# fgiral000/gencast-flax-nnx

Hardware: AMD Instinct MI355X
Metric: denoiser-calls/sec (higher is better)
Workload: dtype f16x3 (every product = 3 fp16 MFMAs on hi/lo-split f32 operands: 22-bit products, f32 accumulate; f32 storage); 1 GPU; nano-GenCast DPM-Solver++2S 20-step sample, 2.5deg grid (73x144), 1 ensemble member per GPU, batch 1; dead_call_skipped=True, grid_nodes=10512, mesh_nodes=2562, latent=256, layers=16, heads=4, ffw_hidden=2048, c_in=262, c_out=82, k_hop=8, parallelism=ensemble-dp1, broadcast=none, rccl_ranks=0, precision=f16x3, library_built_from_this_tree=True, launcher=single

## Files before the change

### gencast-flax-nnx_amd/csrc/gc_api.hip

```cpp
#include <hip/hip_runtime.h>

#include <array>
#include <cmath>
#include <cstdio>
#include <cstdlib>
#include <cstring>
#include <map>
#include <memory>
#include <mutex>
#include <string>
#include <vector>

#include <dlfcn.h>
#include <rccl/rccl.h>

#include "../../include/gencast_hip.h"
#include "../../include/gencast_hip_debug.h"
#include "gc_graph.h"
#include "gc_kernels.h"

template <class To, class From>
static const To& a16_view(const From& v) {
  static_assert(sizeof(To) == sizeof(From), "argument struct mismatch between the two kernel builds");
  return reinterpret_cast<const To&>(v);
// ... 75 lines not shown
  DevMlp m2g_embed_edge, m2g_edge, m2g_grid, m2g_dec;
  std::vector<DevLayer> layers;
  int cond_final = -1;
  int cond_total = 0;
  std::map<std::string, std::pair<int, int>> cond_sites;
  float *d_nw0t = nullptr, *d_nb0 = nullptr, *d_nw1t = nullptr, *d_nb1 = nullptr;
  float *d_wc_all = nullptr, *d_bc_all = nullptr;

  float *d_m0_hat = nullptr, *d_e0_hat = nullptr, *d_f0_hat = nullptr;

  int kp = 0;
  float *d_sigma = nullptr, *d_condvec = nullptr, *d_cond = nullptr;
  float* d_cond_all = nullptr;
  size_t cond_all_cap = 0;
  const float* cond_cur = nullptr;
  float *d_feats = nullptr, *d_xp = nullptr, *d_g0 = nullptr, *d_g1 = nullptr, *d_m0 = nullptr,
        *d_x = nullptr, *d_e1 = nullptr, *d_agg1 = nullptr, *d_qkv = nullptr, *d_att = nullptr,
        *d_u = nullptr, *d_m2 = nullptr, *d_f1 = nullptr, *d_agg2 = nullptr, *d_g2 = nullptr,
        *d_y = nullptr, *d_h = nullptr, *d_part = nullptr, *d_apart_o = nullptr, *d_apart_ml = nullptr,
        *d_pg = nullptr, *d_pm = nullptr;
  bool mlp_ws = true;
  bool mlp_pair = true;
  bool embed_cache = true;
  bool embed_cache_ready = false;
  bool embed_cache_live = false;
  int nwp = 0;
  float *d_xn = nullptr, *d_pstat = nullptr;
  float *w1st_t = nullptr, *w1st_s = nullptr;
  DevMlp g2m_embed_grid_n;
  std::vector<int> h_slots;
  int64_t embed_cache_samples = 0;
  bool mlp_ws512 = true;
  bool m2g_fuse_sum = true;
  bool last_m2g_fused = false;
  float *d_ones = nullptr, *d_zeros = nullptr;
  int hidden_layers = 1;
  float* d_mlp_tmp[2] = {nullptr, nullptr};
  float *d_feats2 = nullptr, *d_ro_a = nullptr, *d_ro_b = nullptr, *d_ro_forc = nullptr;
  int *d_ro_kind = nullptr, *d_ro_src = nullptr, *d_ro_sidx = nullptr;
  int ro_nforc = -1, ro_forc_cap = 0;
  bool has_sample = false;
  int max_tile_chunks = 0;
  int ffw_fused_slabs = 0;
  int ws_mt = 0;
  bool attn_f16 = true;
  bool attn_v2 = true;
  void* d_kv16 = nullptr;
  bool attn_v2_force = false;
  bool kv16_live = false;
  bool fuse_outrow = true;
  bool gemm_ws = true;
  bool f32_ws = true;
  int ffw_xcd = 0;
  bool fuse_combine = true;
  bool split_edge = false;
  int attn_splits = 1, out_splits = 1, ffw2_splits = 1;
  bool a16 = true;
  bool st16 = false;
  bool last_st16 = false;
  int wt_stores = 0;
  int mt_qkv = 1, mt_out = 1, mt_ffw1 = 1, mt_ffw2 = 1;
  int* d_slots = nullptr;
  float *d_sx = nullptr, *d_sden = nullptr, *d_smid = nullptr, *d_noise = nullptr;
  float *d_noise_alt = nullptr, *last_noise = nullptr;
  float* d_stash = nullptr;
  hipEvent_t ev_stash = nullptr;
  bool has_stash = false;

  int nz_L = 0, nz_lat = 0, nz_lon = 0;
  float *d_nz_leg = nullptr, *d_nz_cos = nullptr, *d_nz_sin = nullptr, *d_nz_coef = nullptr, *d_nz_f = nullptr;
  unsigned long long nz_key = 0, nz_stream = 0;
  std::vector<float> churn_rates;
  float churn_inflation = 1.0f;

  struct SampleGraph {
    std::vector<float> sigmas;
    int skip_dead = 1;
    const float* noise = nullptr;
    bool f16 = false, feat16 = false, st16 = false;
    hipGraph_t graph = nullptr;
    hipGraphExec_t exec = nullptr, exec2 = nullptr;
    hipEvent_t done[2] = {nullptr, nullptr};
    int next = 0;
    int calls = 0;
    int64_t launches_per_call = 0, launches = 0;
    uint64_t last_use = 0;
  };
  bool use_graphs = true;
  std::vector<SampleGraph> sample_graphs;
  uint64_t graph_clock = 0;
  int64_t graph_replays = 0, graph_captures = 0;
  int debug_layer_limit = -1;
  int debug_stop_layer = -1, debug_stop_phase = -1;
  bool f16x3 = true;
  float g2m_agg_norm = 0.f;
  bool feat16 = false;
  bool weights_f16_unsafe = false;
  bool in_fallback = false;
  unsigned* d_nonfinite = nullptr;
  unsigned* h_nonfinite = nullptr;
  unsigned nonfinite_seen = 0;
  int64_t range_fallbacks = 0;
  bool guard_pending = false;
  std::vector<float> last_sigmas;
  int last_skip_dead = 1;
  unsigned long long last_stream0 = 0;
// ... 721 lines not shown
      return rc;
    }
    const bool fuse_combine = h->attn_splits > 1 && h->attn_splits <= 8 && h->mt_out == 1 && h->fuse_combine;
    if (h->attn_splits > 1 && !fuse_combine && (rc = launch(h, gc::KC_ATTN_COMBINE, [&] {
          return gc::launch_attn_combine(s, h->d_apart_o, h->d_apart_ml, g.M, B, D, c.num_heads,
                                         h->attn_splits, h->d_att, false, h->feat16);
        })))
      return rc;
    const bool fuse_row = (f16 || x32) && h->gemm_ws && h->fuse_outrow && D % 128 == 0 && D <= 512 &&
                          (h->attn_splits == 1 || fuse_combine);
    if (fuse_row) {
      gc::GemmArgs ga{};
      ga.a = h->d_att; ga.lda = D; ga.a_f32 = 1; ga.wt = x32 ? ly.wo_x : ly.wo_f; ga.ldw = D; ga.rows = MB; ga.n = D; ga.k_slice = D;
      ga.f32w = x32 ? 1 : 0;
      if (h->attn_splits > 1) {
        ga.att_po = h->d_apart_o; ga.att_pml = h->d_apart_ml; ga.att_S = h->attn_splits; ga.att_B = B;
        ga.att_H = c.num_heads; ga.att_DH = D / c.num_heads;
      } else if (use_items) {
        ga.att_po = h->d_apart_o; ga.att_pml = h->d_apart_ml; ga.att_S = 0; ga.att_B = B;
        ga.att_H = c.num_heads; ga.att_DH = D / c.num_heads; ga.att_tiles = h->d_att_tiles;
      }
      ga.round16 = h->feat16 ? 1 : 0; ga.a16 = st16 ? 1 : 0;
      gc::RowFuse rf{h->d_x, ly.bo, cond + ly.cond_ffw, cs, B, h->d_h, h->feat16 ? 1 : 0};
      if ((rc = launch(h, gc::KC_GEMM_OUT, [&] {
             return ga.a16 ? gc_a16::launch_gemm_rowop(s, gc::KC_GEMM_OUT, a16_view<gc_a16::GemmArgs>(ga),
                                                       a16_view<gc_a16::RowFuse>(rf))
                           : gc::launch_gemm_rowop(s, gc::KC_GEMM_OUT, ga, rf);
           })))
        return rc;
    } else if (fuse_combine) {
      gc::GemmArgs ga{};
      const bool ws = use_ws(D, D, h->out_splits);
      ga.a = h->d_att; ga.lda = D; ga.a_f32 = 1; ga.wt = ws ? (x32 ? ly.wo_x : ly.wo_f) : (f16 ? ly.wo_s : ly.wo_t); ga.ldw = D; ga.rows = MB;
      ga.f32w = (ws && x32) ? 1 : 0;
      ga.n = D; ga.k_slice = D / h->out_splits; ga.out = h->d_part; ga.ldo = D;
      ga.att_po = h->d_apart_o; ga.att_pml = h->d_apart_ml; ga.att_S = h->attn_splits; ga.att_B = B;
      ga.att_H = c.num_heads; ga.att_DH = D / c.num_heads; ga.round16 = h->feat16 ? 1 : 0; ga.a16 = st16 ? 1 : 0;
      if ((rc = launch(h, gc::KC_GEMM_OUT, [&] {
             return ws ? (ga.a16 ? gc_a16::launch_gemm_ws(s, gc::KC_GEMM_OUT, a16_view<gc_a16::GemmArgs>(ga), 1, h->out_splits, 1)
                                 : gc::launch_gemm_ws(s, gc::KC_GEMM_OUT, ga, 1, h->out_splits, 1))
                       : gc::launch_gemm(s, gc::KC_GEMM_OUT, ga, 1, h->out_splits, 1, f16);
           })))
        return rc;
    } else if ((rc = gemm(gc::KC_GEMM_OUT, h->d_att, D, f16 ? ly.wo_s : ly.wo_t, x32 ? ly.wo_x : ly.wo_f, D, D, D, h->out_splits,
                          nullptr, 0, h->d_part, D, h->mt_out, 1)))
      return rc;
    if (!fuse_row && (rc = rowop(ly.bo, h->out_splits, ly.cond_ffw, h->d_h))) return rc;
    if (stop_here(i, 2)) return GC_OK;
    if (ffw_slabs > 0) {
      gc::FfwArgs fa{h->d_h, MB, (int)D, (int)F, x32 ? ly.w1_x : ly.w1_f, ly.b1, x32 ? ly.w2_x : ly.w2_f, h->d_part,
                     h->feat16 ? 1 : 0, h->wt_stores & 1, st16 ? 1 : 0};
      fa.f32w = x32 ? 1 : 0;
      fa.xcd_tiles = (h->ffw_xcd && D == 256) ? 1 : 0;
      if ((rc = launch(h, gc::KC_GEMM_FFW1, [&] {
             return fa.a16 ? gc_a16::launch_ffw_fused(s, a16_view<gc_a16::FfwArgs>(fa)) : gc::launch_ffw_fused(s, fa);
           })))
        return rc;
    } else {
    if ((rc = gemm(gc::KC_GEMM_FFW1, h->d_h, D, f16 ? ly.w1_s : ly.w1_t, x32 ? ly.w1_x : ly.w1_f, D, F, D, 1, ly.b1, 1, h->d_u, F,
                   h->mt_ffw1, 0)))
      return rc;
    if ((rc = gemm(gc::KC_GEMM_FFW2, h->d_u, F, f16 ? ly.w2_s : ly.w2_t, x32 ? ly.w2_x : ly.w2_f, F, D, F, h->ffw2_splits, nullptr, 0,
                   h->d_part, D, h->mt_ffw2, 1)))
      return rc;
    }
    pend_bias = ly.b2;
    pend_slabs = ffw_slabs > 0 ? ffw_slabs : h->ffw2_splits;
  }
  if ((rc = rowop(pend_bias, pend_slabs, h->cond_final, h->d_m2))) return rc;

  if (side) GC_HIP(h, hipStreamWaitEvent(s, h->ev_join, 0));
  if (h->split_edge) {
    if ((rc = node_gemm(h->d_m2, g.M * B, h->m2g_edge.w1snd_t, h->m2g_edge.w1snd_s, h->m2g_edge.w1snd_f, h->d_pm))) return rc;
    if ((rc = node_gemm(h->d_g1, g.G * B, h->m2g_edge.w1rcv_t, h->m2g_edge.w1rcv_s, h->m2g_edge.w1rcv_f, h->d_pg))) return rc;
  }
  const bool fuse_sum = m2g_sum_fusable(h);
  h->last_m2g_fused = fuse_sum;
  if ((rc = run_m2g_edge(h, cond, fuse_sum))) return rc;
  if (!fuse_sum && (rc = launch(h, gc::KC_SEGSUM, [&] {
         return gc::launch_segsum(s, h->d_f1, h->d_m2g_ptr, h->d_m2g_eid, g.G, g.E2, B, L, h->d_agg2, h->feat16, st16);
       })))
    return rc;
  if ((rc = run_mlp(h, h->m2g_grid,
                    {seg(h->d_g1, nullptr, nullptr, L, L, 0), seg(h->d_agg2, nullptr, nullptr, L, L, 0)},
                    g.G * B, B, true, true, h->d_g1, h->d_g2, L)))
    return rc;
  if ((rc = run_mlp(h, h->m2g_dec, {seg(h->d_g2, nullptr, nullptr, L, L, 0)}, g.G * B, B, false, false,
                    nullptr, h->d_y, c.c_out, nullptr, nullptr, true, nullptr, false, true)))
    return rc;
  h->launches_last_call = h->launch_count - launches0;
  return GC_OK;
}

int guard_enqueue(gc_handle* h, const float* p, size_t n) {
  if (!use_f16(h)) return GC_OK;
  int rc = launch(h, gc::KC_PACK, [&] { return gc::launch_finite_check(h->stream, p, n, h->d_nonfinite); });
  if (rc) return rc;
  GC_HIP(h, hipMemcpyAsync(h->h_nonfinite, h->d_nonfinite, sizeof(unsigned), hipMemcpyDeviceToHost, h->stream));
  return GC_OK;
}
bool guard_tripped(gc_handle* h) {
  if (*h->h_nonfinite == h->nonfinite_seen) return false;
  h->nonfinite_seen = *h->h_nonfinite;
  return true;
}

// ... 631 lines not shown
    for (int k = 0; k < 4; ++k) e1s[(size_t)e * 32 + k] = g2m_edge_struct[(size_t)e * 4 + k];
  for (int e = 0; e < E2; ++e)
    for (int k = 0; k < 4; ++k) e2s[(size_t)e * 32 + k] = m2g_edge_struct[(size_t)g.m2g_order[e] * 4 + k];
  if ((rc = dev_upload(h, &h->d_mesh_struct16, ms16))) return rc;
  if ((rc = dev_upload(h, &h->d_e1_struct16, e1s))) return rc;
  if ((rc = dev_upload(h, &h->d_e2_struct16, e2s))) return rc;

  const gc_config& c = h->cfg;
  const size_t B = c.batch, L = c.latent_size, D = c.d_model, F = c.ffw_hidden;
  const size_t GB = (size_t)G * B, MB = (size_t)M * B;
  if ((rc = dev_alloc(h, &h->d_sigma, B))) return rc;
  if ((rc = dev_alloc(h, &h->d_condvec, B * gc::kCondDim))) return rc;
  if ((rc = dev_alloc(h, &h->d_feats, GB * c.c_in))) return rc;
  if ((rc = dev_alloc(h, &h->d_xp, GB * h->kp))) return rc;
  if ((rc = dev_alloc(h, &h->d_g0, GB * L))) return rc;
  if ((rc = dev_alloc(h, &h->d_g1, GB * L))) return rc;
  if ((rc = dev_alloc(h, &h->d_g2, GB * L))) return rc;
  if ((rc = dev_alloc(h, &h->d_agg2, GB * L))) return rc;
  if ((rc = dev_alloc(h, &h->d_m0, MB * L))) return rc;
  if ((rc = dev_alloc(h, &h->d_x, MB * L))) return rc;
  if ((rc = dev_alloc(h, &h->d_agg1, MB * L))) return rc;
  if ((rc = dev_alloc(h, &h->d_m2, MB * L))) return rc;
  if ((rc = dev_alloc(h, &h->d_qkv, MB * 3 * D))) return rc;
  if ((rc = dev_alloc(h, &h->d_att, MB * D))) return rc;
  {
    uint16_t* kv = nullptr;
    if ((rc = dev_alloc(h, &kv, MB * 4 * D))) return rc;
    h->d_kv16 = kv;
  }
  if ((rc = dev_alloc(h, &h->d_u, MB * F))) return rc;
  {
    auto env_int = [](const char* name, int dflt) {
      const char* v = std::getenv(name);
      return (v && *v) ? std::atoi(v) : dflt;
    };
    auto largest_split = [](int k, int cap) {
      int best = 1;
      for (int sp = 1; sp <= cap; ++sp)
        if (k % (32 * sp) == 0) best = sp;
      return best;
    };
    int as = (int)std::lround(256.0 / std::max(1, h->hg.n_tiles * (int)B));
    h->attn_splits = std::min(8, std::max(1, env_int("GC_TUNE_ATTN_SPLITS", as)));
    const int ffw2_wgs = (int)((MB + 63) / 64) * (int)(D / 128);
    h->ffw2_splits = largest_split((int)F, std::max(1, env_int("GC_TUNE_FFW2_SPLITS", ffw2_wgs >= 512 ? 1 : 4)));
    h->out_splits = largest_split((int)D, std::max(1, env_int("GC_TUNE_OUT_SPLITS", 2)));
    h->mt_qkv = env_int("GC_TUNE_MT_QKV", 1) == 2 ? 2 : 1;
    h->mt_out = env_int("GC_TUNE_MT_OUT", 1) == 2 ? 2 : 1;
    h->mt_ffw1 = env_int("GC_TUNE_MT_FFW1", 1) == 2 ? 2 : 1;
    h->mt_ffw2 = env_int("GC_TUNE_MT_FFW2", 1) == 2 ? 2 : 1;
    h->fuse_combine = env_int("GC_TUNE_FUSE_COMBINE", 1) != 0;
    h->gemm_ws = env_int("GC_TUNE_GEMM_WS", 1) != 0;
    h->ffw_xcd = env_int("GC_TUNE_FFW_XCD", 0);
    h->f32_ws = env_int("GC_TUNE_F32_WS", 1) != 0 && h->gemm_ws && D % 128 == 0 && F % 256 == 0;
    h->fuse_outrow = env_int("GC_TUNE_FUSE_OUTROW", 1) != 0;
    h->attn_f16 = env_int("GC_TUNE_ATTN_F16", 1) != 0;
    h->attn_v2 = env_int("GC_TUNE_ATTN_V2", 1) != 0;
    h->fuse_noisy = env_int("GC_TUNE_FUSE_NOISY", 1) != 0;
    h->side_stream = env_int("GC_TUNE_SIDE_STREAM", 0) != 0;
    h->wt_stores = env_int("GC_TUNE_WT_STORES", 0);
    h->a16 = env_int("GC_TUNE_A16", 1) != 0;
    h->attn_v2_force = env_int("GC_TUNE_ATTN_V2", 1) == 2;
    h->ws_mt = env_int("GC_TUNE_WS_MT", 0);
    h->mlp_ws = env_int("GC_TUNE_MLP_WS", 1) != 0;
    h->mlp_ws512 = env_int("GC_TUNE_MLP_WS512", 2) != 0;
    h->m2g_fuse_sum = env_int("GC_TUNE_M2G_FUSE_SUM", 1) != 0;
    h->embed_cache = env_int("GC_TUNE_EMBED_CACHE", 1) != 0;
    h->mlp_pair = env_int("GC_TUNE_MLP_PAIR", 1) != 0;
    const int want_fused = env_int("GC_TUNE_FFW_FUSED", 1);
    h->ffw_fused_slabs = (h->gemm_ws && want_fused != 0 && D % 128 == 0 && (D <= 256 || (want_fused == 2 && D <= 512)) &&
                          F % 256 == 0 && F / 256 <= 16) ? (int)(F / 256) : 0;
    const size_t slabs = (size_t)std::max(std::max(h->ffw2_splits, h->out_splits), std::max(h->ffw_fused_slabs, 1));
    if ((rc = dev_alloc(h, &h->d_h, MB * D))) return rc;
    if ((rc = dev_alloc(h, &h->d_pg, GB * L))) return rc;
    if ((rc = dev_alloc(h, &h->d_pm, MB * L))) return rc;
    if (!h->d_ones) {
      if ((rc = dev_upload(h, &h->d_ones, std::vector<float>(2048, 1.0f)))) return rc;
      if ((rc = dev_upload(h, &h->d_zeros, std::vector<float>(2048, 0.0f)))) return rc;
    }
    h->split_edge = env_int("GC_TUNE_SPLIT_EDGE", L >= 512 ? 1 : 0) != 0;
    if ((rc = dev_alloc(h, &h->d_part, slabs * MB * D))) return rc;
    const size_t aslots = (size_t)h->hg.n_tiles * h->attn_splits * B * c.num_heads;
    if ((rc = dev_alloc(h, &h->d_apart_o, aslots * 32 * (D / c.num_heads)))) return rc;
    if ((rc = dev_alloc(h, &h->d_apart_ml, aslots * 32 * 2))) return rc;
  }
  if ((rc = dev_alloc(h, &h->d_e1, (size_t)E1 * B * L))) return rc;
  if ((rc = dev_alloc(h, &h->d_f1, (size_t)E2 * B * L))) return rc;
  if ((rc = dev_alloc(h, &h->d_y, GB * c.c_out))) return rc;
  if ((rc = dev_alloc(h, &h->d_sx, GB * c.c_out))) return rc;
  if ((rc = dev_alloc(h, &h->d_sden, GB * c.c_out))) return rc;
  if ((rc = dev_alloc(h, &h->d_smid, GB * c.c_out))) return rc;
  if ((rc = dev_alloc(h, &h->d_noise, GB * c.c_out))) return rc;
  if ((rc = dev_alloc(h, &h->d_noise_alt, GB * c.c_out))) return rc;
  if ((rc = dev_alloc(h, &h->d_slots, (size_t)c.c_out))) return rc;
  if ((rc = dev_alloc(h, &h->d_m0_hat, (size_t)M * L))) return rc;
  if ((rc = dev_alloc(h, &h->d_e0_hat, (size_t)E1 * L))) return rc;
  if ((rc = dev_alloc(h, &h->d_f0_hat, (size_t)E2 * L))) return rc;
  GC_HIP(h, hipMemset(h->d_xp, 0, GB * h->kp * sizeof(float)));
  GC_HIP(h, hipHostMalloc((void**)&h->pin_cond, GB * c.c_in * sizeof(float), hipHostMallocDefault));
  GC_HIP(h, hipHostMalloc((void**)&h->pin_noise, GB * c.c_out * sizeof(float), hipHostMallocDefault));
  h->has_graph = true;
  h->finalized = false;
  return GC_OK;
  });
}

// ... 906 lines not shown
```

### gencast-flax-nnx_amd/csrc/gc_kernels.hip

```cpp
#include "gc_kernels.h"

#include <algorithm>
#include <atomic>
#include <type_traits>

#include <math.h>
#include <stdlib.h>

#ifdef GC_TU_A16
#define GC_TU_NS gc_a16
#else
#define GC_TU_NS gc
#endif
namespace GC_TU_NS {
#ifdef GC_TU_A16
constexpr bool kTuA16 = true;
#else
constexpr bool kTuA16 = false;
#endif

#include "gc_dev_common.inc"


struct DynLdsOnce {
// ... 388 lines not shown
      }
#pragma unroll
    for (int rr = 0; rr < 8; ++rr) {
      mean[rr] = s1[rr] * inv_n;
      const float var = fmaxf(s2[rr] * inv_n - mean[rr] * mean[rr], 0.f);
      rstd[rr] = 1.0f / sqrtf(var + 1e-6f);
    }
  } else {
#pragma unroll
    for (int rr = 0; rr < 8; ++rr) {
      mean[rr] = 0.f;
      rstd[rr] = 1.f;
    }
  }
#pragma unroll
  for (int rr = 0; rr < 8; ++rr) {
    const int orow = row0 + rbase + rr;
    if (orow >= a.rows) break;
    const float* cs = a.cond ? a.cond + (size_t)(orow % a.B) * a.cond_stride : nullptr;
#pragma unroll
    for (int j = 0; j < CPL; ++j) {
      const int c = lane + 64 * j;
      if (c < n) {
        float v = (yv[rr][j] - mean[rr]) * rstd[rr];
        if (cs) v = v * cs[c] + cs[n + c];
        a.out[(size_t)orow * a.ldo + c] = r16_if(r16_if(v, a.round_out) + rv[rr][j], a.round_out);
      }
    }
  }
}

template <class T>
__device__ __forceinline__ T pick3(int i, T x0, T x1, T x2) {
  T v = x2;
  if (i == 1) v = x1;
  if (i == 0) v = x0;
  return v;
}

template <int NT, int R>
__device__ __forceinline__ void ws_ring_fill(f32x4 (&wh)[R][NT], f32x4 (&wl)[R][NT], const float* wf,
                                             size_t ct_stride, int steps_total) {
#pragma unroll
  for (int j = 0; j < R; ++j) {
    const int sn = j < steps_total ? j : steps_total - 1;
#pragma unroll
    for (int nt = 0; nt < NT; ++nt) {
      wh[j][nt] = ld4(wf + nt * ct_stride + (size_t)sn * 512);
      wl[j][nt] = ld4(wf + nt * ct_stride + (size_t)sn * 512 + 256);
    }
  }
}

template <int MT, int NT, int R, int J0, bool A16 = false, bool F32 = false>
__device__ __forceinline__ void ws_quad(f32x16 (&acc)[MT][NT], f32x16 (&acc2)[MT][NT], f32x4 (&wh)[R][NT],
                                        f32x4 (&wl)[R][NT], const float* a_row, int mt_stride, int kstep0,
                                        const float* wf, size_t ct_stride, int& s, int steps_total) {
#pragma unroll
  for (int j = 0; j < 4; ++j) {
    const int kk = kstep0 + j;
    const int off = F32 ? kk * 16 : (kk >> 1) * 32 + (kk & 1) * 8;
#pragma unroll
    for (int mt = 0; mt < MT; ++mt) {
      if constexpr (F32) {
        const f32x4 a0 = ld4(a_row + mt * mt_stride + off), a1 = ld4(a_row + mt * mt_stride + off + 4);
#pragma unroll
        for (int e = 0; e < 4; ++e)
#pragma unroll
          for (int nt = 0; nt < NT; ++nt) acc[mt][nt] = mfma32(wh[J0 + j][nt][e], a0[e], acc[mt][nt]);
#pragma unroll
        for (int e = 0; e < 4; ++e)
#pragma unroll
          for (int nt = 0; nt < NT; ++nt) acc[mt][nt] = mfma32(wl[J0 + j][nt][e], a1[e], acc[mt][nt]);
        continue;
      }
      const f32x4 ah = ld4(a_row + mt * mt_stride + off);
      f32x4 al;
      if constexpr (!A16) al = ld4(a_row + mt * mt_stride + off + 16);
#pragma unroll
      for (int nt = 0; nt < NT; ++nt) acc2[mt][nt] = mfma16(wl[J0 + j][nt], ah, acc2[mt][nt]);
#pragma unroll
      for (int nt = 0; nt < NT; ++nt) acc[mt][nt] = mfma16(wh[J0 + j][nt], ah, acc[mt][nt]);
      if constexpr (!A16) {
#pragma unroll
        for (int nt = 0; nt < NT; ++nt) acc2[mt][nt] = mfma16(wh[J0 + j][nt], al, acc2[mt][nt]);
      }
    }
    __builtin_amdgcn_sched_barrier(0);
    int sn = s + R;
    if (sn >= steps_total) sn = steps_total - 1;
#pragma unroll
    for (int nt = 0; nt < NT; ++nt) {
      wh[J0 + j][nt] = ld4(wf + nt * ct_stride + (size_t)sn * 512);
      wl[J0 + j][nt] = ld4(wf + nt * ct_stride + (size_t)sn * 512 + 256);
    }
    ++s;
    __builtin_amdgcn_sched_barrier(0);
  }
}

__device__ __forceinline__ void ln_accumulate(const f32x4& y, float& s1, float& s2) {
#pragma unroll
  for (int e = 0; e < 4; ++e) {
    s1 += y[e];
    s2 = __builtin_fmaf(y[e], y[e], s2);
  }
}
__device__ __forceinline__ void ln_finish(float s1, float s2, float inv_n, float& mean, float& rstd) {
  mean = s1 * inv_n;
  const float var = fmaxf(__builtin_fmaf(-mean, mean, s2 * inv_n), 0.f);
  rstd = 1.0f / sqrtf(var + 1e-6f);
}
__device__ __forceinline__ f32x4 ln_affine(const f32x4& y, float mean, float rstd, const f32x4& sc, const f32x4& of) {
  f32x4 r;
#pragma unroll
  for (int e = 0; e < 4; ++e) r[e] = __builtin_fmaf((y[e] - mean) * rstd, sc[e], of[e]);
  return r;
}

template <int NT1, int WM, int NWC>
constexpr int mlp_ws_occ() { return NWC >= 8 ? (NT1 == 1 ? 4 : 2) : ((WM >= 2 || NT1 >= 4) ? 1 : 2); }
template <int NT1, int NT2, int MT, int WM, int NWC, int NW2, int OCC, bool A16, bool F32>
__device__ __forceinline__ void gc_mlp_ws_body(const MlpArgs& a, const int bid) {
  static_assert(!(A16 && F32), "one or the other");
  extern __shared__ __attribute__((aligned(16))) float smem[];
  constexpr int HID = NT1 * 32 * NWC, NPAD = NT2 * 32 * NW2, BM = 32 * MT * WM, NTHR = 64 * NWC * WM;
  constexpr int KC = BM >= 128 ? 64 : 128, LDA = KC + 4, LDH = HID + 4, LDY = NPAD + 4;
  constexpr int PPR = KC / 4;
  constexpr int RSTEP = NTHR / PPR;
  constexpr int AP = BM / RSTEP;
  constexpr int R1 = (OCC < 4 && (NT1 * MT <= 2 || (NT1 >= 4 && MT == 1))) ? 8 : 4;
  constexpr int R2 = (OCC < 4 && (NT2 * MT <= 2 || (NT1 >= 4 && NT2 * MT <= 4))) ? 8 : 4;
  int* srcoff = reinterpret_cast<int*>(smem);
  int* srcb = srcoff + 3 * BM;
  int* addoff = srcb + BM;
  float* region = smem + 6 * BM;

  const int tid = threadIdx.x;
  const int wave_all = tid >> 6, lane = tid & 63, r = lane & 31, hh = lane >> 5;
  const int wave = wave_all % NWC, wrow = (wave_all / NWC) * (MT * 32);
  const int row0 = bid * BM;
  constexpr int TPB = BM / 3;
  const int tri = a.tri;
  const int unit0 = bid * TPB, units = a.rows / 3;
  const int w0 = a.seg[0].width, w1 = a.nseg > 1 ? a.seg[1].width : 0, w2 = a.nseg > 2 ? a.seg[2].width : 0;
  const int ktot = w0 + w1 + w2, kpad = a.k1f;

  const float *p0 = a.seg[0].ptr, *p1 = a.seg[1].ptr, *p2 = a.seg[2].ptr;
  const float *f0 = a.seg[0].affine, *f1 = a.nseg > 1 ? a.seg[1].affine : nullptr,
              *f2 = a.nseg > 2 ? a.seg[2].affine : nullptr;
  {
// ... 1862 lines not shown

template <int CLS>
static hipError_t launch_gemm_rowop_c(hipStream_t s, const GemmArgs& g, const RowFuse& f) {
  const int D = g.n;
  if (D % 128 || D > 512 || g.k_slice != D || g.ldw != D || !f.x || !f.h || !f.cond || f.B < 1 ||
      g.att_S > kMaxAttnSplits)
    return hipErrorInvalidValue;
  const int nt = D > 256 ? 2 : 1;
  const int nthr = (D / (32 * nt)) * 64;
  static int rh_env = -1;
  if (rh_env < 0) {
    const char* e = getenv("GC_TUNE_OUT_RH");
    rh_env = (e && *e) ? atoi(e) : 0;
  }
  const int t32 = (g.rows + 31) / 32, t48 = (g.rows + 47) / 48;
  int rh = t32 <= 128 ? 16 : 32;
  if (t32 > 256 && (t32 + 255) / 256 > (t48 + 255) / 256 && nthr == 512 && g.att_S == 0) rh = 48;
  if (rh_env == 16 || rh_env == 32 || (rh_env == 48 && nthr == 512 && g.att_S == 0)) rh = rh_env;
  const size_t lds = (size_t)(rh > 32 ? 64 : 32) * (D + 4) * sizeof(float);
  const int grid = (g.rows + rh - 1) / rh;
  if (grid <= 0) return hipSuccess;
#define GC_ROWOP_R(NT_, AM_, RH_)                                                                          \
  {                                                                                                        \
    if constexpr (!kTuA16) {                                                                               \
      if (g.f32w) {                                                                                        \
        static DynLdsOnce once32;                                                                          \
        if (hipError_t e = once32.ensure((const void*)gc_gemm_rowop_kernel<NT_, AM_, CLS, RH_, false, true>, 64 * 516 * 4)) return e; \
        hipLaunchKernelGGL((gc_gemm_rowop_kernel<NT_, AM_, CLS, RH_, false, true>), dim3(grid), dim3(nthr), lds, s, g, f); \
        return hipGetLastError();                                                                          \
      }                                                                                                    \
    }                                                                                                      \
    static DynLdsOnce once;                                                                                \
    if (hipError_t e = once.ensure((const void*)gc_gemm_rowop_kernel<NT_, AM_, CLS, RH_, kTuA16>, 64 * 516 * 4)) return e; \
    hipLaunchKernelGGL((gc_gemm_rowop_kernel<NT_, AM_, CLS, RH_, kTuA16>), dim3(grid), dim3(nthr), lds, s, g, f); \
  }
#define GC_ROWOP(NT_, AM_) { if (rh == 16) GC_ROWOP_R(NT_, AM_, 16) else if (rh == 48 && AM_ == 0) GC_ROWOP_R(NT_, 0, 48) else GC_ROWOP_R(NT_, AM_, 32) }
  if (nt == 1 && g.att_S > 0) GC_ROWOP(1, 1)
  else if (nt == 1) GC_ROWOP(1, 0)
  else if (g.att_S > 0) GC_ROWOP(2, 1)
  else GC_ROWOP(2, 0)
#undef GC_ROWOP
#undef GC_ROWOP_R
  return hipGetLastError();
}

hipError_t launch_gemm_rowop(hipStream_t s, int cls, const GemmArgs& g, const RowFuse& f) {
  switch (cls) {
    case KC_GEMM_OUT: return launch_gemm_rowop_c<KC_GEMM_OUT>(s, g, f);
    default: return hipErrorInvalidValue;
  }
}

template <int ND, int MT, int NWC = 4, bool A16 = false ,
          bool F32 = false >
__global__ __launch_bounds__(64 * NWC, NWC == 8 ? 2 : ((ND <= 2 && MT == 1) ? 3 : (ND * MT <= 4 ? 2 : 1))) void gc_ffw_fused_kernel(FfwArgs g) {
  extern __shared__ __attribute__((aligned(16))) float smem[];
  constexpr int D = 128 * ND, LDA = D + 4, FS = 256, LDU = FS + 4, R = 4, BM = 32 * MT;
  constexpr int NTHR = 64 * NWC, NT1 = FS / (32 * NWC), NT2 = D / (32 * NWC);
  constexpr int AP = 32 * (D / 4) / NTHR;
  float* At = smem;
  float* Ut = smem;
  const int tid = threadIdx.x, wave = tid >> 6, lane = tid & 63, r = lane & 31, hh = lane >> 5;
  const int S = g.f / FS;
  int z = blockIdx.x % S, mtile = blockIdx.x / S;
  if (g.xcd_tiles) {
    const int xcd = blockIdx.x & 7, j = blockIdx.x >> 3;
    mtile = (j / S) * 8 + xcd;
    z = j - (j / S) * S;
    if (mtile * BM >= g.rows) return;
  }
#ifdef GC_STAMPS
  unsigned long long stamp_v[8];
  int stamp_n = 0;
#define GC_STAMP() do { stamp_v[stamp_n++] = __builtin_amdgcn_s_memtime(); } while (0)
#else
#define GC_STAMP() do { } while (0)
#endif
  GC_STAMP();

  constexpr int steps1 = D / 16;
  const float* wf1 = g.w1f + (size_t)(z * (FS / 32) + wave * NT1) * steps1 * 512 + lane * 4;
  f32x4 wh1[R][NT1], wl1[R][NT1];
  ws_ring_fill<NT1, R>(wh1, wl1, wf1, (size_t)steps1 * 512, steps1);

  if constexpr (A16) {
    static_assert(AP % 2 == 0, "fp16 piece mapping");
    f32x4 ra[MT][AP / 2];
#pragma unroll
    for (int mb = 0; mb < MT; ++mb)
#pragma unroll
      for (int i = 0; i < AP / 2; ++i) {
        const int p = tid + NTHR * i, row = mb * 32 + p / (D / 8), c8 = p % (D / 8);
        int grow = mtile * BM + row;
        if (grow >= g.rows) grow = g.rows - 1;
        ra[mb][i] = ld4(reinterpret_cast<const float*>(as_h16(g.a) + (size_t)grow * D + c8 * 8));
      }
#pragma unroll
    for (int mb = 0; mb < MT; ++mb)
#pragma unroll
      for (int i = 0; i < AP / 2; ++i) {
        const int p = tid + NTHR * i, row = mb * 32 + p / (D / 8), c8 = p % (D / 8);
        st4(At + row * LDA + (c8 >> 2) * 32 + (c8 & 3) * 4, ra[mb][i]);
      }
  } else {
    f32x4 ra[MT][AP];
#pragma unroll
    for (int mb = 0; mb < MT; ++mb)
#pragma unroll
      for (int i = 0; i < AP; ++i) {
        const int p = tid + NTHR * i, row = mb * 32 + p / (D / 4), c4 = p % (D / 4);
        int grow = mtile * BM + row;
        if (grow >= g.rows) grow = g.rows - 1;
        ra[mb][i] = ld4(g.a + (size_t)grow * D + c4 * 4);
      }
#pragma unroll
    for (int mb = 0; mb < MT; ++mb)
#pragma unroll
      for (int i = 0; i < AP; ++i) {
        const int p = tid + NTHR * i, row = mb * 32 + p / (D / 4), c4 = p % (D / 4);
        if constexpr (F32) st4(At + row * LDA + c4 * 4, ra[mb][i]);
        else stage16<A16>(At + row * LDA + (c4 >> 3) * 32, c4 & 7, ra[mb][i]);
      }
  }
  GC_STAMP();
  __syncthreads();
  GC_STAMP();

  constexpr bool kB1Early = NWC == 8;
  f32x4 b1pre[kB1Early ? NT1 : 1][4];
  if constexpr (kB1Early) {
#pragma unroll
    for (int nt = 0; nt < NT1; ++nt)
#pragma unroll
      for (int j = 0; j < 4; ++j) b1pre[nt][j] = ld4(g.b1 + z * FS + (wave * NT1 + nt) * 32 + 4 * hh + 8 * j);
  }

  f32x16 acc1[MT][NT1], accx1[MT][NT1];
#pragma unroll
  for (int mt = 0; mt < MT; ++mt)
#pragma unroll
    for (int nt = 0; nt < NT1; ++nt)
#pragma unroll
      for (int q = 0; q < 16; ++q) {
        acc1[mt][nt][q] = 0.f;
        accx1[mt][nt][q] = 0.f;
      }
  {
    int s = 0;
    const float* arow = At + r * LDA + hh * (F32 ? 8 : 4);
#pragma unroll 1
    for (int st = 0; st < steps1; st += 4)
      ws_quad<MT, NT1, R, 0, A16, F32>(acc1, accx1, wh1, wl1, arow, 32 * LDA, st, wf1, (size_t)steps1 * 512, s, steps1);
  }
  GC_STAMP();
  const int steps2_total = g.f / 16;
  const float* wf2 = g.w2f + ((size_t)(wave * NT2) * steps2_total + (size_t)z * (FS / 16)) * 512 + lane * 4;
  const size_t cts2 = (size_t)steps2_total * 512;
  f32x4 wh2[R][NT2], wl2[R][NT2];
  ws_ring_fill<NT2, R>(wh2, wl2, wf2, cts2, FS / 16);

  typedef _Float16 f16x4 __attribute__((ext_vector_type(4)));
  typedef float f32x2v __attribute__((ext_vector_type(2)));
  f16x4 uh[NT1][4][MT], ul[NT1][4][MT];
  with_flag(g.round16, [&](auto rc) __attribute__((always_inline)) {
    constexpr bool RND = decltype(rc)::value;
#pragma unroll
    for (int nt = 0; nt < NT1; ++nt) {
      const int cbase = (wave * NT1 + nt) * 32 + 4 * hh;
#pragma unroll
      for (int j = 0; j < 4; ++j) {
        f32x4 bv;
        if constexpr (kB1Early) bv = b1pre[nt][j];
        else bv = ld4(g.b1 + z * FS + cbase + 8 * j);
#pragma unroll
        for (int mt = 0; mt < MT; ++mt) {
          _Float16 hv[4], lv[4];
          if constexpr (F32) {
            f32x4 uf;
#pragma unroll
            for (int e = 0; e < 4; ++e) uf[e] = r16_c<RND>(gelu_tanh_fast(acc1[mt][nt][4 * j + e] + bv[e]));
            uh[nt][j][mt] = __builtin_bit_cast(f16x4, f32x2v{uf[0], uf[1]});
            ul[nt][j][mt] = __builtin_bit_cast(f16x4, f32x2v{uf[2], uf[3]});
            continue;
          }
#pragma unroll
          for (int e = 0; e < 4; ++e) {
            const float u = r16_c<RND>(gelu_tanh_fast(hilo(acc1[mt][nt][4 * j + e], accx1[mt][nt][4 * j + e]) + bv[e]));
            if constexpr (A16) {
              hv[e] = (_Float16)u;
              lv[e] = (_Float16)0.f;
            } else {
              split16(u, hv[e], lv[e]);
            }
          }
          uh[nt][j][mt] = f16x4{hv[0], hv[1], hv[2], hv[3]};
          ul[nt][j][mt] = f16x4{lv[0], lv[1], lv[2], lv[3]};
        }
      }
    }
  });
  __syncthreads();
#pragma unroll
  for (int nt = 0; nt < NT1; ++nt) {
    const int cbase = (wave * NT1 + nt) * 32 + 4 * hh;
#pragma unroll
    for (int j = 0; j < 4; ++j)
#pragma unroll
      for (int mt = 0; mt < MT; ++mt) {
        const int col = cbase + 8 * j;
        if constexpr (F32) {
          float* pf = Ut + (size_t)(mt * 32 + r) * LDU + col;
          *reinterpret_cast<f16x4*>(pf) = uh[nt][j][mt];
          *reinterpret_cast<f16x4*>(pf + 2) = ul[nt][j][mt];
          continue;
        }
        _Float16* p = reinterpret_cast<_Float16*>(Ut + (size_t)(mt * 32 + r) * LDU + (col & ~31)) + (col & 31);
        *reinterpret_cast<f16x4*>(p) = uh[nt][j][mt];
        if constexpr (!A16) *reinterpret_cast<f16x4*>(p + 32) = ul[nt][j][mt];
      }
  }
  __syncthreads();
  GC_STAMP();

  f32x16 acc2[MT][NT2], accx2[MT][NT2];
#pragma unroll
  for (int mt = 0; mt < MT; ++mt)
#pragma unroll
    for (int nt = 0; nt < NT2; ++nt)
#pragma unroll
      for (int q = 0; q < 16; ++q) {
        acc2[mt][nt][q] = 0.f;
        accx2[mt][nt][q] = 0.f;
      }
  {
    int s = 0;
    const float* urow = Ut + r * LDU + hh * (F32 ? 8 : 4);
#pragma unroll 1
    for (int st = 0; st < FS / 16; st += 4)
      ws_quad<MT, NT2, R, 0, A16, F32>(acc2, accx2, wh2, wl2, urow, 32 * LDU, st, wf2, cts2, s, FS / 16);
  }
  GC_STAMP();
#pragma unroll
  for (int mt = 0; mt < MT; ++mt) {
    const int grow = mtile * BM + mt * 32 + r;
    if (grow >= g.rows) continue;
    float* orow = g.out + ((size_t)z * g.rows + grow) * D;
#pragma unroll
    for (int nt = 0; nt < NT2; ++nt) {
      const int cbase = (wave * NT2 + nt) * 32 + 4 * hh;
#pragma unroll
      for (int j = 0; j < 4; ++j) {
        f32x4 v;
#pragma unroll
        for (int e = 0; e < 4; ++e) v[e] = hilo(acc2[mt][nt][4 * j + e], accx2[mt][nt][4 * j + e]);
        if (g.wt) st4_wt(orow + cbase + 8 * j, v);
        else st4(orow + cbase + 8 * j, v);
      }
    }
  }
#ifdef GC_STAMPS
  GC_STAMP();
  asm volatile("s_waitcnt vmcnt(0)" ::: "memory");
  GC_STAMP();
  if (g.stamps && lane == 0)
    for (int i = 0; i < 8; ++i) g.stamps[((size_t)blockIdx.x * NWC + wave) * 8 + i] = stamp_v[i];
#endif
#undef GC_STAMP
}

template <int ND, int MT, int NWC = 4>
static hipError_t launch_ffw_fused_t(hipStream_t s, const FfwArgs& g) {
  const size_t lds = (size_t)(32 * MT * ((ND > 2 ? 128 * ND : 256) + 4)) * sizeof(float);
  const int n_mt = (g.rows + 32 * MT - 1) / (32 * MT);
  const int grid = g.xcd_tiles ? 8 * ((n_mt + 7) / 8) * (g.f / 256) : n_mt * (g.f / 256);
  if (grid <= 0) return hipSuccess;
  if constexpr (!kTuA16) {
    if (g.f32w) {
      static DynLdsOnce once32;
      if (hipError_t e = once32.ensure((const void*)gc_ffw_fused_kernel<ND, MT, NWC, false, true>, (int)lds)) return e;
      hipLaunchKernelGGL((gc_ffw_fused_kernel<ND, MT, NWC, false, true>), dim3(grid), dim3(64 * NWC), lds, s, g);
      return hipGetLastError();
    }
  }
  static DynLdsOnce once;
  if (hipError_t e = once.ensure((const void*)gc_ffw_fused_kernel<ND, MT, NWC, kTuA16>, (int)lds)) return e;
  hipLaunchKernelGGL((gc_ffw_fused_kernel<ND, MT, NWC, kTuA16>), dim3(grid), dim3(64 * NWC), lds, s, g);
  return hipGetLastError();
}

hipError_t launch_ffw_fused(hipStream_t s, const FfwArgs& g) {
  if (g.d % 128 || g.d > 512 || g.f % 256 || g.f < 256) return hipErrorInvalidValue;
  static int mt2 = -1;
  if (mt2 < 0) {
    const char* e = getenv("GC_TUNE_FFW_MT");
    mt2 = e ? atoi(e) : 0;
  }
  const bool big = mt2 == 2 || (mt2 == 0 && ((g.rows + 63) / 64) * (g.f / 256) >= 300);
  switch (g.d / 128) {
    case 1: return big ? launch_ffw_fused_t<1, 2>(s, g) : launch_ffw_fused_t<1, 1>(s, g);
    case 2: {
      const int b96 = ((g.rows + 95) / 96) * (g.f / 256);
      if (mt2 == 38 || (mt2 == 0 && b96 > 128 && b96 <= 256)) return launch_ffw_fused_t<2, 3, 8>(s, g);
      if (mt2 == 28) return launch_ffw_fused_t<2, 2, 8>(s, g);
      return big ? launch_ffw_fused_t<2, 2>(s, g) : launch_ffw_fused_t<2, 1>(s, g);
    }
    case 4: return launch_ffw_fused_t<4, 1>(s, g);
    default: return hipErrorInvalidValue;
  }
}

hipError_t launch_gemm_ws(hipStream_t s, int cls, const GemmArgs& g, int mt, int splits, int epi) {
  switch (cls) {
    case KC_GEMM_QKV: return launch_gemm_ws_c<KC_GEMM_QKV>(s, g, mt, splits, epi);
    case KC_GEMM_OUT: return launch_gemm_ws_c<KC_GEMM_OUT>(s, g, mt, splits, epi);
    case KC_GEMM_FFW1: return launch_gemm_ws_c<KC_GEMM_FFW1>(s, g, mt, splits, epi);
    case KC_GEMM_FFW2: return launch_gemm_ws_c<KC_GEMM_FFW2>(s, g, mt, splits, epi);
    case KC_GEMM_NODE: return launch_gemm_ws_c<KC_GEMM_NODE>(s, g, mt, splits, epi);
    default: return hipErrorInvalidValue;
  }
}

hipError_t launch_gemm(hipStream_t s, int cls, const GemmArgs& g, int shape, int splits, int epi, bool f16) {
  switch (cls) {
    case KC_GEMM_QKV: return launch_gemm_c<KC_GEMM_QKV>(s, g, shape, splits, epi, f16);
    case KC_GEMM_OUT: return launch_gemm_c<KC_GEMM_OUT>(s, g, shape, splits, epi, f16);
    case KC_GEMM_FFW1: return launch_gemm_c<KC_GEMM_FFW1>(s, g, shape, splits, epi, f16);
    case KC_GEMM_FFW2: return launch_gemm_c<KC_GEMM_FFW2>(s, g, shape, splits, epi, f16);
    case KC_GEMM_NODE: return launch_gemm_c<KC_GEMM_NODE>(s, g, shape, splits, epi, f16);
    default: return hipErrorInvalidValue;
  }
}

template <int NS , bool H16 = false>
// ... 1010 lines not shown
```

### gencast-flax-nnx_amd/csrc/gc_kernels_decl.inc

```
namespace GC_KERNELS_NS {

enum KernelClass : int {
  KC_COND = 0,
  KC_PACK,
  KC_MLP,
  KC_SEGSUM,
  KC_ROWOP,
  KC_GEMM_QKV,
  KC_ATTN,
  KC_ATTN_COMBINE,
  KC_GEMM_OUT,
  KC_GEMM_FFW1,
  KC_GEMM_FFW2,
  KC_GEMM_NODE,
  KC_NOISE,
  KC_COUNT
};

constexpr int kTileM = 32;
constexpr int kCondDim = 16;

struct Segment {
  const float* ptr;
  const int* index;
// ... 61 lines not shown

hipError_t launch_mlp(hipStream_t s, const MlpArgs& a);
bool mlp_pair_supported(const MlpArgs& a, const MlpArgs& b);
hipError_t launch_mlp_pair(hipStream_t s, const MlpArgs& a, const MlpArgs& b);

hipError_t launch_segsum(hipStream_t s, const float* src, const int* rowptr, const int* eids,
                         int n_items, int n_edges, int B, int width, float* out, bool round16 = false,
                         bool h16 = false ,
                         float norm = 0.f );

struct GemmArgs {
  const float* a;
  int lda;
  int a_f32;
  const float* att_po;
  const float* att_pml;
  int att_S, att_B, att_H, att_DH;
  const int* att_tiles;
  const float* wt;
  int ldw;
  int rows, n;
  int k_slice;
  int splits;
  const float* bias;
  int act;
  float* out;
  int ldo;
  int round16;
  int a16;
  void* kv16;
  int kv_d;
  int out_f32;
  int f32w;
};
hipError_t launch_gemm(hipStream_t s, int cls, const GemmArgs& g, int shape, int splits, int epi, bool f16);
hipError_t launch_gemm_ws(hipStream_t s, int cls, const GemmArgs& g, int mt, int splits, int epi);
#ifdef GC_STAMPS
hipError_t set_gemm_ws_stamp_buffer(unsigned long long* p);
#endif

struct FfwArgs {
  const float* a;
  int rows, d, f;
  const float* w1f;
  const float* b1;
  const float* w2f;
  float* out;
  int round16;
  int wt;
  int a16;
  unsigned long long* stamps;
  int f32w;
  int xcd_tiles;
};
hipError_t launch_ffw_fused(hipStream_t s, const FfwArgs& g);

struct RowFuse {
  float* x;
  const float* bias;
  const float* cond;
  int cond_stride;
  int B;
  float* h;
  int round16;
};
hipError_t launch_gemm_rowop(hipStream_t s, int cls, const GemmArgs& g, const RowFuse& f);
#ifdef GC_STAMPS
hipError_t set_gemm_rowop_stamp_buffer(unsigned long long* p);
#endif

hipError_t launch_rowop(hipStream_t s, float* x, const float* bias, const float* partials, int n_slabs,
                        int rows, int d, int B, const float* cond, int cond_stride, float* h,
                        int h_s16 ,
                        bool round16 = false, bool h16 = false ,
                        int xcd_tile_rows = 0 );

hipError_t launch_attention(hipStream_t s, const float* qkv, float* o, float* part_o, float* part_ml,
                            int M, int B, int D, int H, int S, bool out_s16,
                            const int* tile_chunk_start, const int* union_idx, const unsigned* mask_bits,
                            int n_tiles, bool f16 = false, int max_chunks_per_tile = 0, bool feat16 = false,
                            const int* items = nullptr , int n_items = 0);
hipError_t launch_attention_v2(hipStream_t s, const float* qkv, const void* kv16, float* o, float* part_o,
                               float* part_ml, int M, int B, int D, int H, int S, const int* tile_chunk_start,
                               const int* union_idx, const unsigned* mask_bits, int n_tiles,
                               int max_chunks_per_tile, bool feat16,
                               bool h16 = false ,
                               const int* items = nullptr ,
                               int n_items = 0);
#ifdef GC_STAMPS
hipError_t set_attention_stamp_buffer(unsigned long long* p);
#endif
hipError_t launch_attn_combine(hipStream_t s, const float* part_o, const float* part_ml, int M, int B,
                               int D, int H, int S, float* o, bool out_s16, bool round16 = false);

hipError_t launch_pack_full(hipStream_t s, const float* grid_struct, const float* feats, int G, int B,
                            int c_in, int kp, float* xp);
hipError_t launch_write_noisy(hipStream_t s, const float* x, const int* slots, int rows, int c_out,
                              int kp, float scale, float* xp);
hipError_t launch_write_noisy_compact(hipStream_t s, const float* x, int rows, int c_out, int ldn, float scale, float* xn);
hipError_t launch_zero_slots(hipStream_t s, const int* slots, int rows, int c_out, int kp, float* xp);
hipError_t launch_affine_rows(hipStream_t s, const float* src, const float* cond, int cond_stride,
                              int items, int B, int w, float* out, bool round16 = false,
                              bool h16 = false );
hipError_t launch_finite_check(hipStream_t s, const float* p, size_t n, unsigned* counter);
constexpr int kItemPieces = 4;
struct NoisyWrite {
  const int* slots = nullptr;
// ... 26 lines not shown
```

Measured before the change: 784.0 calls/s.

## Pipeline fused FFW kernel with chunked A staging and per-wave LDS flags

```diff
diff --git a/gencast-flax-nnx_amd/csrc/gc_api.hip b/gencast-flax-nnx_amd/csrc/gc_api.hip
--- a/gencast-flax-nnx_amd/csrc/gc_api.hip
+++ b/gencast-flax-nnx_amd/csrc/gc_api.hip
@@ -151,6 +151,7 @@
   bool gemm_ws = true;
   bool f32_ws = true;
   int ffw_xcd = 0;
+  int ffw_pipe = 1;
   bool fuse_combine = true;
   bool split_edge = false;
   int attn_splits = 1, out_splits = 1, ffw2_splits = 1;
@@ -978,6 +979,7 @@
                      h->feat16 ? 1 : 0, h->wt_stores & 1, st16 ? 1 : 0};
       fa.f32w = x32 ? 1 : 0;
       fa.xcd_tiles = (h->ffw_xcd && D == 256) ? 1 : 0;
+      fa.pipe = h->ffw_pipe;
       if ((rc = launch(h, gc::KC_GEMM_FFW1, [&] {
              return fa.a16 ? gc_a16::launch_ffw_fused(s, a16_view<gc_a16::FfwArgs>(fa)) : gc::launch_ffw_fused(s, fa);
            })))
@@ -1715,6 +1717,7 @@
     h->fuse_combine = env_int("GC_TUNE_FUSE_COMBINE", 1) != 0;
     h->gemm_ws = env_int("GC_TUNE_GEMM_WS", 1) != 0;
     h->ffw_xcd = env_int("GC_TUNE_FFW_XCD", 0);
+    h->ffw_pipe = env_int("GC_TUNE_FFW_PIPE", 1);
     h->f32_ws = env_int("GC_TUNE_F32_WS", 1) != 0 && h->gemm_ws && D % 128 == 0 && F % 256 == 0;
     h->fuse_outrow = env_int("GC_TUNE_FUSE_OUTROW", 1) != 0;
     h->attn_f16 = env_int("GC_TUNE_ATTN_F16", 1) != 0;
diff --git a/gencast-flax-nnx_amd/csrc/gc_kernels.hip b/gencast-flax-nnx_amd/csrc/gc_kernels.hip
--- a/gencast-flax-nnx_amd/csrc/gc_kernels.hip
+++ b/gencast-flax-nnx_amd/csrc/gc_kernels.hip
@@ -464,51 +464,57 @@
   }
 }
 
+template <int NS, int MT, int NT, int R, int J0, bool A16 = false, bool F32 = false>
+__device__ __forceinline__ void ws_steps(f32x16 (&acc)[MT][NT], f32x16 (&acc2)[MT][NT], f32x4 (&wh)[R][NT],
+                                         f32x4 (&wl)[R][NT], const float* a_row, int mt_stride, int kstep0,
+                                         const float* wf, size_t ct_stride, int& s, int steps_total) {
+#pragma unroll
+  for (int j = 0; j < NS; ++j) {
+    const int kk = kstep0 + j;
+    const int off = F32 ? kk * 16 : (kk >> 1) * 32 + (kk & 1) * 8;
+#pragma unroll
+    for (int mt = 0; mt < MT; ++mt) {
+      if constexpr (F32) {
+        const f32x4 a0 = ld4(a_row + mt * mt_stride + off), a1 = ld4(a_row + mt * mt_stride + off + 4);
+#pragma unroll
+        for (int e = 0; e < 4; ++e)
+#pragma unroll
+          for (int nt = 0; nt < NT; ++nt) acc[mt][nt] = mfma32(wh[J0 + j][nt][e], a0[e], acc[mt][nt]);
+#pragma unroll
+        for (int e = 0; e < 4; ++e)
+#pragma unroll
+          for (int nt = 0; nt < NT; ++nt) acc[mt][nt] = mfma32(wl[J0 + j][nt][e], a1[e], acc[mt][nt]);
+        continue;
+      }
+      const f32x4 ah = ld4(a_row + mt * mt_stride + off);
+      f32x4 al;
+      if constexpr (!A16) al = ld4(a_row + mt * mt_stride + off + 16);
+#pragma unroll
+      for (int nt = 0; nt < NT; ++nt) acc2[mt][nt] = mfma16(wl[J0 + j][nt], ah, acc2[mt][nt]);
+#pragma unroll
+      for (int nt = 0; nt < NT; ++nt) acc[mt][nt] = mfma16(wh[J0 + j][nt], ah, acc[mt][nt]);
+      if constexpr (!A16) {
+#pragma unroll
+        for (int nt = 0; nt < NT; ++nt) acc2[mt][nt] = mfma16(wh[J0 + j][nt], al, acc2[mt][nt]);
+      }
+    }
+    __builtin_amdgcn_sched_barrier(0);
+    int sn = s + R;
+    if (sn >= steps_total) sn = steps_total - 1;
+#pragma unroll
+    for (int nt = 0; nt < NT; ++nt) {
+      wh[J0 + j][nt] = ld4(wf + nt * ct_stride + (size_t)sn * 512);
+      wl[J0 + j][nt] = ld4(wf + nt * ct_stride + (size_t)sn * 512 + 256);
+    }
+    ++s;
+    __builtin_amdgcn_sched_barrier(0);
+  }
+}
 template <int MT, int NT, int R, int J0, bool A16 = false, bool F32 = false>
 __device__ __forceinline__ void ws_quad(f32x16 (&acc)[MT][NT], f32x16 (&acc2)[MT][NT], f32x4 (&wh)[R][NT],
                                         f32x4 (&wl)[R][NT], const float* a_row, int mt_stride, int kstep0,
                                         const float* wf, size_t ct_stride, int& s, int steps_total) {
-#pragma unroll
-  for (int j = 0; j < 4; ++j) {
-    const int kk = kstep0 + j;
-    const int off = F32 ? kk * 16 : (kk >> 1) * 32 + (kk & 1) * 8;
-#pragma unroll
-    for (int mt = 0; mt < MT; ++mt) {
-      if constexpr (F32) {
-        const f32x4 a0 = ld4(a_row + mt * mt_stride + off), a1 = ld4(a_row + mt * mt_stride + off + 4);
-#pragma unroll
-        for (int e = 0; e < 4; ++e)
-#pragma unroll
-          for (int nt = 0; nt < NT; ++nt) acc[mt][nt] = mfma32(wh[J0 + j][nt][e], a0[e], acc[mt][nt]);
-#pragma unroll
-        for (int e = 0; e < 4; ++e)
-#pragma unroll
-          for (int nt = 0; nt < NT; ++nt) acc[mt][nt] = mfma32(wl[J0 + j][nt][e], a1[e], acc[mt][nt]);
-        continue;
-      }
-      const f32x4 ah = ld4(a_row + mt * mt_stride + off);
-      f32x4 al;
-      if constexpr (!A16) al = ld4(a_row + mt * mt_stride + off + 16);
-#pragma unroll
-      for (int nt = 0; nt < NT; ++nt) acc2[mt][nt] = mfma16(wl[J0 + j][nt], ah, acc2[mt][nt]);
-#pragma unroll
-      for (int nt = 0; nt < NT; ++nt) acc[mt][nt] = mfma16(wh[J0 + j][nt], ah, acc[mt][nt]);
-      if constexpr (!A16) {
-#pragma unroll
-        for (int nt = 0; nt < NT; ++nt) acc2[mt][nt] = mfma16(wh[J0 + j][nt], al, acc2[mt][nt]);
-      }
-    }
-    __builtin_amdgcn_sched_barrier(0);
-    int sn = s + R;
-    if (sn >= steps_total) sn = steps_total - 1;
-#pragma unroll
-    for (int nt = 0; nt < NT; ++nt) {
-      wh[J0 + j][nt] = ld4(wf + nt * ct_stride + (size_t)sn * 512);
-      wl[J0 + j][nt] = ld4(wf + nt * ct_stride + (size_t)sn * 512 + 256);
-    }
-    ++s;
-    __builtin_amdgcn_sched_barrier(0);
-  }
+  ws_steps<4, MT, NT, R, J0, A16, F32>(acc, acc2, wh, wl, a_row, mt_stride, kstep0, wf, ct_stride, s, steps_total);
 }
 
 __device__ __forceinline__ void ln_accumulate(const f32x4& y, float& s1, float& s2) {
@@ -2477,12 +2483,15 @@
 }
 
 template <int ND, int MT, int NWC = 4, bool A16 = false ,
-          bool F32 = false >
+          bool F32 = false ,
+          bool PIPE = false>
 __global__ __launch_bounds__(64 * NWC, NWC == 8 ? 2 : ((ND <= 2 && MT == 1) ? 3 : (ND * MT <= 4 ? 2 : 1))) void gc_ffw_fused_kernel(FfwArgs g) {
   extern __shared__ __attribute__((aligned(16))) float smem[];
   constexpr int D = 128 * ND, LDA = D + 4, FS = 256, LDU = FS + 4, R = 4, BM = 32 * MT;
   constexpr int NTHR = 64 * NWC, NT1 = FS / (32 * NWC), NT2 = D / (32 * NWC);
   constexpr int AP = 32 * (D / 4) / NTHR;
+  static_assert(!PIPE || (ND == 2 && MT == 3 && NWC == 8 && !F32), "pipelined schedule: the 96-row d = 256 form only");
+  constexpr int LDX = 36, GX = BM * LDX, XOFF = BM * LDA, FLAGOFF = XOFF + 4 * GX;
   float* At = smem;
   float* Ut = smem;
   const int tid = threadIdx.x, wave = tid >> 6, lane = tid & 63, r = lane & 31, hh = lane >> 5;
@@ -2495,19 +2504,86 @@
     if (mtile * BM >= g.rows) return;
   }
 #ifdef GC_STAMPS
-  unsigned long long stamp_v[8];
+  unsigned long long stamp_v[kFfwStampWords] = {};
   int stamp_n = 0;
 #define GC_STAMP() do { stamp_v[stamp_n++] = __builtin_amdgcn_s_memtime(); } while (0)
 #else
 #define GC_STAMP() do { } while (0)
 #endif
   GC_STAMP();
+  if constexpr (PIPE) {
+    if ((g.pipe & 2) && __builtin_amdgcn_readfirstlane(tid) >= 256) __builtin_amdgcn_s_setprio(1);
+  }
 
   constexpr int steps1 = D / 16;
   const float* wf1 = g.w1f + (size_t)(z * (FS / 32) + wave * NT1) * steps1 * 512 + lane * 4;
   f32x4 wh1[R][NT1], wl1[R][NT1];
   ws_ring_fill<NT1, R>(wh1, wl1, wf1, (size_t)steps1 * 512, steps1);
 
+  constexpr bool kB1Early = NWC == 8;
+  f32x4 b1pre[kB1Early ? NT1 : 1][4];
+  f32x16 acc1[MT][NT1], accx1[MT][NT1];
+
+  if constexpr (PIPE) {
+    constexpr int NCH = A16 ? 2 : 4, QPC = 4 / NCH;
+    int* flags = reinterpret_cast<int*>(smem + FLAGOFF);
+    if (tid < 8) flags[tid] = 0;
+    f32x4 ra[NCH][MT];
+#pragma unroll
+    for (int c = 0; c < NCH; ++c)
+#pragma unroll
+      for (int mb = 0; mb < MT; ++mb) {
+        int grow = mtile * BM + mb * 32 + (tid >> 4);
+        if (grow >= g.rows) grow = g.rows - 1;
+        const int cp = c * 16 + (tid & 15);
+        if constexpr (A16) ra[c][mb] = ld4(reinterpret_cast<const float*>(as_h16(g.a) + (size_t)grow * D + cp * 8));
+        else ra[c][mb] = ld4(g.a + (size_t)grow * D + cp * 4);
+      }
+#pragma unroll
+    for (int nt = 0; nt < NT1; ++nt)
+#pragma unroll
+      for (int j = 0; j < 4; ++j) b1pre[nt][j] = ld4(g.b1 + z * FS + (wave * NT1 + nt) * 32 + 4 * hh + 8 * j);
+    auto stage_chunk = [&](int c) __attribute__((always_inline)) {
+#pragma unroll
+      for (int mb = 0; mb < MT; ++mb) {
+        const int row = mb * 32 + (tid >> 4), cp = c * 16 + (tid & 15);
+        if constexpr (A16) st4(At + row * LDA + (cp >> 2) * 32 + (cp & 3) * 4, ra[c][mb]);
+        else stage16<A16>(At + row * LDA + (cp >> 3) * 32, cp & 7, ra[c][mb]);
+      }
+    };
+    stage_chunk(0);
+    GC_STAMP();
+    __syncthreads();
+    GC_STAMP();
+#pragma unroll
+    for (int mt = 0; mt < MT; ++mt)
+#pragma unroll
+      for (int nt = 0; nt < NT1; ++nt)
+#pragma unroll
+        for (int q = 0; q < 16; ++q) {
+          acc1[mt][nt][q] = 0.f;
+          accx1[mt][nt][q] = 0.f;
+        }
+    int s = 0;
+    const float* arow = At + r * LDA + hh * 4;
+#pragma unroll
+    for (int c = 0; c < NCH; ++c) {
+#pragma unroll
+      for (int q = 0; q < QPC; ++q)
+        ws_quad<MT, NT1, R, 0, A16, F32>(acc1, accx1, wh1, wl1, arow, 32 * LDA, (c * QPC + q) * 4, wf1, (size_t)steps1 * 512, s,
+                                         steps1);
+      if (c + 1 < NCH) {
+        stage_chunk(c + 1);
+#ifdef GC_STAMPS
+        const unsigned long long tb = __builtin_amdgcn_s_memtime();
+#endif
+        __syncthreads();
+#ifdef GC_STAMPS
+        stamp_v[10] += __builtin_amdgcn_s_memtime() - tb;
+#endif
+      }
+    }
+  } else {
   if constexpr (A16) {
     static_assert(AP % 2 == 0, "fp16 piece mapping");
     f32x4 ra[MT][AP / 2];
@@ -2551,8 +2627,6 @@
   __syncthreads();
   GC_STAMP();
 
-  constexpr bool kB1Early = NWC == 8;
-  f32x4 b1pre[kB1Early ? NT1 : 1][4];
   if constexpr (kB1Early) {
 #pragma unroll
     for (int nt = 0; nt < NT1; ++nt)
@@ -2560,7 +2634,6 @@
       for (int j = 0; j < 4; ++j) b1pre[nt][j] = ld4(g.b1 + z * FS + (wave * NT1 + nt) * 32 + 4 * hh + 8 * j);
   }
 
-  f32x16 acc1[MT][NT1], accx1[MT][NT1];
 #pragma unroll
   for (int mt = 0; mt < MT; ++mt)
 #pragma unroll
@@ -2576,6 +2649,7 @@
 #pragma unroll 1
     for (int st = 0; st < steps1; st += 4)
       ws_quad<MT, NT1, R, 0, A16, F32>(acc1, accx1, wh1, wl1, arow, 32 * LDA, st, wf1, (size_t)steps1 * 512, s, steps1);
+  }
   }
   GC_STAMP();
   const int steps2_total = g.f / 16;
@@ -2624,6 +2698,22 @@
       }
     }
   });
+  GC_STAMP();
+  if constexpr (PIPE) {
+    const int wv = __builtin_amdgcn_readfirstlane(wave);
+    float* grp = wv < 4 ? Ut + wv * 32 : smem + XOFF + (wv - 4) * GX;
+    const int ldg = wv < 4 ? LDU : LDX;
+#pragma unroll
+    for (int j = 0; j < 4; ++j)
+#pragma unroll
+      for (int mt = 0; mt < MT; ++mt) {
+        _Float16* p = reinterpret_cast<_Float16*>(grp + (size_t)(mt * 32 + r) * ldg) + 4 * hh + 8 * j;
+        *reinterpret_cast<f16x4*>(p) = uh[0][j][mt];
+        if constexpr (!A16) *reinterpret_cast<f16x4*>(p + 32) = ul[0][j][mt];
+      }
+    asm volatile("s_waitcnt lgkmcnt(0)" ::: "memory");
+    if (lane == 0) __hip_atomic_store(reinterpret_cast<int*>(smem + FLAGOFF) + wv, 1, __ATOMIC_RELAXED, __HIP_MEMORY_SCOPE_WORKGROUP);
+  } else {
   __syncthreads();
 #pragma unroll
   for (int nt = 0; nt < NT1; ++nt) {
@@ -2645,6 +2735,7 @@
       }
   }
   __syncthreads();
+  }
   GC_STAMP();
 
   f32x16 acc2[MT][NT2], accx2[MT][NT2];
@@ -2657,7 +2748,29 @@
         acc2[mt][nt][q] = 0.f;
         accx2[mt][nt][q] = 0.f;
       }
-  {
+  if constexpr (PIPE) {
+    int s = 0;
+    const int* flags = reinterpret_cast<const int*>(smem + FLAGOFF);
+    auto group = [&](int gi, auto j0) __attribute__((always_inline)) {
+#ifdef GC_STAMPS
+      const unsigned long long tw = __builtin_amdgcn_s_memtime();
+#endif
+      while (__builtin_amdgcn_readfirstlane(__hip_atomic_load(flags + gi, __ATOMIC_RELAXED, __HIP_MEMORY_SCOPE_WORKGROUP)) == 0)
+        __builtin_amdgcn_s_sleep(1);
+      asm volatile("" ::: "memory");
+#ifdef GC_STAMPS
+      stamp_v[9] += __builtin_amdgcn_s_memtime() - tw;
+#endif
+      const float* urow = (gi < 4 ? Ut + gi * 32 + r * LDU : smem + XOFF + (gi - 4) * GX + r * LDX) + hh * 4;
+      ws_steps<2, MT, NT2, R, decltype(j0)::value, A16, F32>(acc2, accx2, wh2, wl2, urow, 32 * (gi < 4 ? LDU : LDX), 0, wf2,
+                                                             cts2, s, FS / 16);
+    };
+#pragma unroll
+    for (int gp = 0; gp < 8; gp += 2) {
+      group(gp, std::integral_constant<int, 0>{});
+      group(gp + 1, std::integral_constant<int, 2>{});
+    }
+  } else {
     int s = 0;
     const float* urow = Ut + r * LDU + hh * (F32 ? 8 : 4);
 #pragma unroll 1
@@ -2688,7 +2801,7 @@
   asm volatile("s_waitcnt vmcnt(0)" ::: "memory");
   GC_STAMP();
   if (g.stamps && lane == 0)
-    for (int i = 0; i < 8; ++i) g.stamps[((size_t)blockIdx.x * NWC + wave) * 8 + i] = stamp_v[i];
+    for (int i = 0; i < kFfwStampWords; ++i) g.stamps[((size_t)blockIdx.x * NWC + wave) * kFfwStampWords + i] = stamp_v[i];
 #endif
 #undef GC_STAMP
 }
@@ -2704,6 +2817,15 @@
       static DynLdsOnce once32;
       if (hipError_t e = once32.ensure((const void*)gc_ffw_fused_kernel<ND, MT, NWC, false, true>, (int)lds)) return e;
       hipLaunchKernelGGL((gc_ffw_fused_kernel<ND, MT, NWC, false, true>), dim3(grid), dim3(64 * NWC), lds, s, g);
+      return hipGetLastError();
+    }
+  }
+  if constexpr (ND == 2 && MT == 3 && NWC == 8) {
+    if (g.pipe & 1) {
+      const size_t lds_p = lds + (size_t)(4 * 96 * 36 + 8) * sizeof(float);
+      static DynLdsOnce once_p;
+      if (hipError_t e = once_p.ensure((const void*)gc_ffw_fused_kernel<ND, MT, NWC, kTuA16, false, true>, (int)lds_p)) return e;
+      hipLaunchKernelGGL((gc_ffw_fused_kernel<ND, MT, NWC, kTuA16, false, true>), dim3(grid), dim3(64 * NWC), lds_p, s, g);
       return hipGetLastError();
     }
   }
diff --git a/gencast-flax-nnx_amd/csrc/gc_kernels_decl.inc b/gencast-flax-nnx_amd/csrc/gc_kernels_decl.inc
--- a/gencast-flax-nnx_amd/csrc/gc_kernels_decl.inc
+++ b/gencast-flax-nnx_amd/csrc/gc_kernels_decl.inc
@@ -137,7 +137,9 @@
   unsigned long long* stamps;
   int f32w;
   int xcd_tiles;
-};
+  int pipe;
+};
+constexpr int kFfwStampWords = 12;
 hipError_t launch_ffw_fused(hipStream_t s, const FfwArgs& g);
 
 struct RowFuse {
```

Result: no change. 785.8 calls/s (median of 6 runs) (+0.2%).
